# basilevh/tcow

Measured on AMD Instinct MI355X. Metric: train clips/sec (T=30, 240x320), higher is better.
Workload: dtype bf16; 1 GPU; TCOW Seeker train step: T=30 240x320 patch16, 12-layer divided space-time ViT (D=768), num_queries=3, causal_attention=1, 1 clip/GPU; clips_per_gpu=1, num_queries=3, parallelism=dp1, optimizer=AdamW lr 1e-4, clip 0.3

## Files before the change

### include/tcow_hip.h

```cpp
#ifndef TCOW_HIP_H
#define TCOW_HIP_H

#ifdef __cplusplus
extern "C" {
#endif

#define TCOW_OK 0
#define TCOW_ERR_INVALID_ARG (-1)
#define TCOW_ERR_LAUNCH (-2)
#define TCOW_ERR_UNSUPPORTED (-3)

#define TCOW_F32 0
#define TCOW_BF16 1
#define TCOW_F32X3 2

#define TCOW_ACT_NONE 0
#define TCOW_ACT_GELU 1
#define TCOW_ACT_DGELU 2
#define TCOW_ACT_GELU_DSAVE 3
#define TCOW_ACT_MUL_AUX 4

#define TCOW_ABI_VERSION 14
int tcow_version(void);
const char* tcow_last_error(void);
// ... 166 lines not shown
int tcow_droppath_rows(void* stream, int depth, int B, int T, int S, const float* u, const float* keep_p, const float* mask0, float* out);
int tcow_cast_transpose(void* stream, int dtype, int N, int K, const float* W, void* Wc, void* Wt);
long tcow_cast_desc_bytes(void);
int tcow_cast_transpose_batched(void* stream, int dtype, const void* table, int n, int total_tiles);

long tcow_adamw_chunk_bytes(void);
int tcow_adamw_clip_step(void* stream, const void* chunks, int n_chunks, float lr, float beta1, float beta2, float eps,
                         float weight_decay, int step, float max_norm, float* scratch);
int tcow_adamw_clip_step_scaled(void* stream, const void* chunks, int n_chunks, float lr, float beta1, float beta2, float eps,
                                float weight_decay, int step, float max_norm, float* scratch, const float* grad_inv_scale);
long tcow_adamw_tile_bytes(void);
int tcow_adamw_clip_step_cast(void* stream, const void* chunks, int n_chunks, const void* flat_chunks, int n_flat, const void* tiles, int n_tiles, float lr, float beta1,
                              float beta2, float eps, float weight_decay, int step, float max_norm, float* scratch, const float* grad_inv_scale);

typedef struct {
    long n_frames, frame_len, frames_per_seq;
    const float* logits;  long logits_seq_stride;
    const float* target;  long target_seq_stride;
    const float* pixel_w;
    const float* frame_w;
    int weighted_aot;
    float aot_loss;
    double topk_frac;
    float loss_weight;
    float* loss;
    float* total;
    float* dlogits;  long dlogits_seq_stride;
    void* ws;  size_t ws_bytes;
    int focal;
} tcow_mask_loss_args;
size_t tcow_mask_loss_workspace_bytes(long n_frames, long frame_len);
size_t tcow_mask_loss_workspace_bytes_for(long n_frames, long frame_len, double topk_frac, float aot_loss);
int tcow_mask_loss(void* stream, const tcow_mask_loss_args* args);
int tcow_mask_loss_batch(void* stream, const tcow_mask_loss_args* args, int n);

int tcow_iou_counts(void* stream, const float* logits, const float* target, long n_frames, long frame_len, int* counts);

int tcow_build_masks(void* stream, int B, int Q, int M, int T, long HW, int query_time, const unsigned char* segm,
                     const unsigned char* div_segm, const int* query_idx, const int* front_idx, const int* cont_idx,
                     float* query_mask, float* target_mask, unsigned char* snitch_occl_by_ptr, int* counts);

int tcow_build_query_masks(void* stream, int B, int Q, int K, int M, int T, long HW, int query_time, const unsigned char* segm,
                           const unsigned char* div_segm, const float* occl_fracs, const float* dag, const long long* sel, float front_thres,
                           float front_half_thres, float outer_thres, float occluded_weight, float zero_weight, float has_weight, int* idx_ws,
                           unsigned char* ids, float* flags, float* sel_occl_fracs, float* frame_w, float* query_mask, float* target_mask,
                           unsigned char* snitch_occl_by_ptr, int* counts);

int tcow_iou_means(void* stream, const int* counts, int n_seq, int C, int T, float* mean, int* count);

size_t tcow_snitch_weights_workspace_bytes(long n_frames, int H, int W);
int tcow_snitch_weights(void* stream, long n_seq, int T, int H, int W, const float* target_ch0, long target_seq_stride,
                        const unsigned char* snitch_occl_by_ptr, const float* frame_w, const int* pos_count, int class_balancing,
                        float hard_negative_factor, float* weights, void* ws, size_t ws_bytes);

#ifdef __cplusplus
}
#endif
#endif
```

### tcow_amd/_lib.py

```python
import ctypes
import os

_HERE = os.path.dirname(os.path.abspath(__file__))
LIB_PATH = os.environ.get('TCOW_LIB') or os.path.join(_HERE, 'libtcow_hip.so')
LIB_PATH_FP16 = os.path.join(_HERE, 'libtcow_hip_fp16.so')

TCOW_F32, TCOW_BF16, TCOW_F32X3 = 0, 1, 2
TCOW_FP8E4M3 = 3
ACT_NONE, ACT_GELU, ACT_DGELU, ACT_GELU_DSAVE, ACT_MUL_AUX = 0, 1, 2, 3, 4


class TcowError(RuntimeError):
    """Raised when a libtcow_hip entry point returns a non-zero status (message from tcow_last_error)."""


class AttnShape(ctypes.Structure):
    _fields_ = [('B', ctypes.c_int), ('T', ctypes.c_int), ('S', ctypes.c_int), ('D', ctypes.c_int),
                ('heads', ctypes.c_int), ('causal', ctypes.c_int), ('dtype', ctypes.c_int)]


class GemmArgs(ctypes.Structure):
    _fields_ = [('M', ctypes.c_int), ('N', ctypes.c_int), ('K', ctypes.c_int), ('dtype', ctypes.c_int),
                ('A', ctypes.c_void_p), ('lda', ctypes.c_long), ('W', ctypes.c_void_p), ('ldw', ctypes.c_long),
                ('C', ctypes.c_void_p), ('ldc', ctypes.c_long), ('out_f32', ctypes.c_int),
# ... 84 lines not shown
    'tcow_im2col': (_i, [_vp, _i, _i, _i, _i, _i, _i, _vp, _vp, _i, _vp]),
    'tcow_gather_frames': (_i, [_vp, _i, _i, _i, _i, _i, _i, _i, _i, _vp, _vp, _vp, _vp, _vp]),
    'tcow_resize_aa': (_i, [_vp, _i, _i, _i, _i, _i, _i, _i, _i, _i, _vp, _vp, _vp, _vp, _vp, _vp, _vp, _i, _vp, _vp, _vp, _i, _vp]),
    'tcow_photometric_workspace_bytes': (_l, [_i]),
    'tcow_photometric': (_i, [_vp, _i, _i, _i, _i, _i, _i, _i, _i, _vp, _vp, _i, ctypes.POINTER(ctypes.c_int), _f, _f, _f, _f, _i, ctypes.POINTER(ctypes.c_float), _i,
                         _vp, _l, _vp]),
    'tcow_im2col_channels': (_i, [_vp, _i, _i, _i, _i, _i, _i, _i, _vp, _i, _vp]),
    'tcow_col2im': (_i, [_vp, _i, _i, _i, _i, _i, _vp, _l, _vp, _vp, _i, _vp]),
    'tcow_col2im_channels': (_i, [_vp, _i, _i, _i, _i, _i, _i, _vp, _l, _i, _vp, _vp]),
    'tcow_embed_fwd': (_i,[_vp, _i, _i, _i, _i, _vp, _vp, _vp, _vp]),
    'tcow_embed_bwd': (_i, [_vp, _i, _i, _i, _i, _vp, _vp, _vp, _i]),
    'tcow_cls_merge': (_i, [_vp, _i, _i, _i, _i, _vp, _i, _i]),
    'tcow_cls_merge_bwd_cast': (_i, [_vp, _i, _i, _i, _i, _i, _vp, _i, _vp, _l, _vp]),
    'tcow_unpatchify_pool_fwd': (_i, [_vp, _i, _i, _i, _i, _i, _i, _i, _vp, _vp]),
    'tcow_unpatchify_pool_bwd': (_i, [_vp, _i, _i, _i, _i, _i, _i, _i, _vp, _vp]),
    'tcow_upsample_fwd': (_i, [_vp, _i, _i, _i, _i, _i, _i, _i, _vp, _vp]),
    'tcow_upsample_bwd': (_i, [_vp, _i, _i, _i, _i, _i, _i, _i, _vp, _vp]),
    'tcow_upsample_bwd_amax': (_i, [_vp, _i, _i, _i, _i, _i, _i, _vp, _vp, _vp, _i]),
    'tcow_flags_fwd': (_i, [_vp, _i, _i, _i, _i, _vp, _vp, _vp, _vp]),
    'tcow_droppath_rows': (_i, [_vp, _i, _i, _i, _i, _vp, _vp, _vp, _vp]),
    'tcow_scale_cast': (_i, [_vp, _i, _l, _i, _vp, _l, _vp, _vp, _l]),
    'tcow_scale_unless_one': (_i, [_vp, _vp, _l, _vp]),
    'tcow_cast_transpose': (_i, [_vp, _i, _i, _i, _vp, _vp, _vp]),
    'tcow_cast_desc_bytes': (_l, []),
    'tcow_cast_transpose_batched': (_i, [_vp, _i, _vp, _i, _i]),
    'tcow_adamw_chunk_bytes': (_l, []),
    'tcow_adamw_clip_step': (_i, [_vp, _vp, _i, _f, _f, _f, _f, _f, _i, _f, _vp]),
    'tcow_adamw_clip_step_scaled': (_i, [_vp, _vp, _i, _f, _f, _f, _f, _f, _i, _f, _vp, _vp]),
    'tcow_adamw_tile_bytes': (_l, []),
    'tcow_adamw_clip_step_cast': (_i, [_vp, _vp, _i, _vp, _i, _vp, _i, _f, _f, _f, _f, _f, _i, _f, _vp, _vp]),
    'tcow_mask_loss_workspace_bytes': (ctypes.c_size_t, [_l, _l]),
    'tcow_mask_loss_workspace_bytes_for': (ctypes.c_size_t, [_l, _l, ctypes.c_double, _f]),
    'tcow_mask_loss': (_i, [_vp, ctypes.POINTER(MaskLossArgs)]),
    'tcow_mask_loss_batch': (_i, [_vp, ctypes.POINTER(MaskLossArgs), _i]),
    'tcow_iou_counts': (_i, [_vp, _vp, _vp, _l, _l, _vp]),
    'tcow_build_masks': (_i, [_vp, _i, _i, _i, _i, _l, _i, _vp, _vp, _vp, _vp, _vp, _vp, _vp, _vp, _vp]),
    'tcow_build_query_masks': (_i, [_vp, _i, _i, _i, _i, _i, _l, _i, _vp, _vp, _vp, _vp, _vp, _f, _f, _f, _f, _f, _f, _vp, _vp, _vp, _vp, _vp, _vp, _vp, _vp, _vp]),
    'tcow_iou_means': (_i, [_vp, _vp, _i, _i, _i, _vp, _vp]),
    'tcow_snitch_weights_workspace_bytes': (ctypes.c_size_t, [_l, _i, _i]),
    'tcow_snitch_weights': (_i, [_vp, _l, _i, _i, _i, _vp, _l, _vp, _vp, _vp, _i, _f, _vp, _vp, ctypes.c_size_t]),
}


ABI_VERSION = 14


def _declare(L, tolerant=False):
    for name, (res, args) in SIGNATURES.items():
        if tolerant and not hasattr(L, name):
            continue
        fn = getattr(L, name)
        fn.restype = res
        fn.argtypes = args



def lib(fmt='bf16'):
    L = _libs.get(fmt)
    if L is None:
        path = LIB_PATH if fmt == 'bf16' else LIB_PATH_FP16
        if not os.path.exists(path):
            raise TcowError(f'{path} not found: build it with `make` (or __graft_entry__.build()); '
                            'the Seeker HIP path has no fallback')
        import torch
        L = ctypes.CDLL(path)
        L.tcow_last_error.restype = ctypes.c_char_p
# ... 12 lines not shown
```

### tcow_amd/csrc/mask_loss.hip

```cpp
#include "common.h"

namespace {

constexpr int kThreads = 256;
constexpr int kVecPerBlock = 1024;
constexpr int kBins12 = 2048, kBins3 = 512;
constexpr int kNPart = 6;

struct MlView {
    const float* x; long xs;
    const float* t; long ts;
    const float* pw;
    const float* fw;
    float* dx; long dxs;
    int T; int L4; int n_frames; int weighted;
    int focal;
};

struct MlCtl {
    long n_sel, n_all, k, above, cnt_eq, r;
    int valid, mode_all, jac_valid, pad;
    unsigned b1, b2, tau, pad2;
    double S[kNPart];
    double topk_sum;
};

struct MlWs {
    int* fsel; double* fwsum; double* part; unsigned* hist; MlCtl* ctl; int nblk;
    unsigned* vb;
};

constexpr int kMaxJobs = 4;
struct MlJob { MlView v; MlWs ws; float aot, lw; double topk_frac; float* loss; int radix; };
struct MlBatch { int n; float* total; MlJob j[kMaxJobs]; };

__device__ __forceinline__ void bce_sig(float x, float t, float& bce, float& p) {
    const float e = expf(-fabsf(x));
    const float inv = 1.0f / (1.0f + e);
    p = x >= 0.0f ? inv : e * inv;
    bce = fmaxf(x, 0.0f) - x * t + log1pf(e);
}

__device__ __forceinline__ void pix_loss(float x, float t, int focal, float& val, float& dval, float& p) {
    float bce; bce_sig(x, t, bce, p);
    if (!focal) { val = bce; dval = p - t; return; }
    const float pt = p * t + (1.0f - p) * (1.0f - t), at = 0.25f * t + 0.75f * (1.0f - t), q = 1.0f - pt;
    val = at * bce * (q * q);
    dval = at * q * (q * (p - t) - 2.0f * p * (1.0f - p) * (2.0f * t - 1.0f) * bce);
}

__device__ __forceinline__ double block_sum(double v, double* red) {
    for (int o = 32; o > 0; o >>= 1) v += __shfl_xor(v, o, 64);
    const int w = threadIdx.x >> 6;
    __syncthreads();
    if ((threadIdx.x & 63) == 0) red[w] = v;
    __syncthreads();
    double s = 0.0;
    for (int i = 0; i < kThreads / 64; ++i) s += red[i];
    return s;
}

__device__ __forceinline__ long elem_off(const MlView& v, int f, long stride) {
    const int s = f / v.T;
    return (long)s * stride + (long)(f - s * v.T) * v.L4 * 4;
}

__device__ __forceinline__ void ml_frames_body(const MlView& v, const MlWs& ws) {
    __shared__ double red[kThreads / 64];
    const int f = blockIdx.x;
    const float fwv = v.fw ? v.fw[f] : 1.0f;
    double sum = 0.0; int any = 0;
    if (v.pw) {
        const float4* pw = reinterpret_cast<const float4*>(v.pw + (long)f * v.L4 * 4);
        float s = 0.f;
        for (int i = threadIdx.x; i < v.L4; i += kThreads) {
            float4 w = pw[i];
            w.x *= fwv; w.y *= fwv; w.z *= fwv; w.w *= fwv;
            any |= (w.x != 0.f) | (w.y != 0.f) | (w.z != 0.f) | (w.w != 0.f);
            s += (w.x + w.y) + (w.z + w.w);
        }
        sum = s;
    } else if (threadIdx.x == 0) {
        any = fwv != 0.f; sum = (double)fwv * (v.L4 * 4.0);
    }
    sum = block_sum(sum, red);
    any = __syncthreads_or(any);
    if (threadIdx.x == 0) { ws.fsel[f] = any; ws.fwsum[f] = sum; }
}

__device__ __forceinline__ void ml_ctl_body(const MlView& v, const MlWs& ws, double topk_frac) {
    __shared__ double red[kThreads / 64];
    double nf = 0.0, wsum = 0.0;
    for (int f = threadIdx.x; f < v.n_frames; f += kThreads) { nf += ws.fsel[f] ? 1.0 : 0.0; wsum += ws.fwsum[f]; }
    nf = block_sum(nf, red); wsum = block_sum(wsum, red);
    for (int i = threadIdx.x; i < 2 * kBins12 + kBins3; i += kThreads) ws.hist[i] = 0u;
    if (threadIdx.x == 0) {
        MlCtl c = {};
        c.n_all = (long)v.n_frames * v.L4 * 4;
        c.n_sel = (long)nf * v.L4 * 4;
        const float wmean = (float)(wsum / (double)c.n_all);
        c.valid = c.n_sel > 0 && wmean >= 1e-4f;
        c.k = (long)(topk_frac * (double)c.n_sel);
        c.mode_all = c.k >= c.n_sel;
        *ws.ctl = c;
    }
}

template <typename F> __device__ __forceinline__ void for_each_vec(const MlView& v, int f, F&& fn) {
    const float4* x = reinterpret_cast<const float4*>(v.x + elem_off(v, f, v.xs));
    const float4* t = reinterpret_cast<const float4*>(v.t + elem_off(v, f, v.ts));
    const float4* pw = v.pw ? reinterpret_cast<const float4*>(v.pw + (long)f * v.L4 * 4) : nullptr;
    const float fwv = v.fw ? v.fw[f] : 1.0f;
    const int base = blockIdx.x * kVecPerBlock;
#pragma unroll
    for (int j = 0; j < kVecPerBlock / kThreads; ++j) {
        const int i = base + j * kThreads + threadIdx.x;
        if (i < v.L4) {
            float4 w = pw ? pw[i] : make_float4(1.f, 1.f, 1.f, 1.f);
            w.x *= fwv; w.y *= fwv; w.z *= fwv; w.w *= fwv;
            fn(x[i], t[i], w, i);
        }
    }
}

__device__ __forceinline__ unsigned vbits(float bce, float w, int weighted) {
    const unsigned u = __builtin_bit_cast(unsigned, weighted ? bce * w : bce);
    return (int)u < 0 ? 0u : u;
}

__device__ __forceinline__ void ml_stats_body(const MlView& v, const MlWs& ws, int radix) {
    __shared__ unsigned hist[kBins12];
    __shared__ double red[kThreads / 64];
    const int f = blockIdx.y;
    const MlCtl* c = ws.ctl;
    const bool live = c->valid && ws.fsel[f];
    const bool need_hist = live && !c->mode_all && radix;
    if (need_hist) { for (int i = threadIdx.x; i < kBins12; i += kThreads) hist[i] = 0u; }
    __syncthreads();
    float s[5] = {0.f, 0.f, 0.f, 0.f, 0.f};
    if (live) {
        uint4* vbo = need_hist ? reinterpret_cast<uint4*>(ws.vb + (long)f * v.L4 * 4) : nullptr;
        for_each_vec(v, f, [&](float4 x, float4 t, float4 w, int i) {
            const float xs[4] = {x.x, x.y, x.z, x.w}, ts[4] = {t.x, t.y, t.z, t.w}, wv[4] = {w.x, w.y, w.z, w.w};
            unsigned vbs[4];
#pragma unroll
            for (int e = 0; e < 4; ++e) {
                float bce, dval, p; pix_loss(xs[e], ts[e], v.focal, bce, dval, p);
                const unsigned vb = vbits(bce, wv[e], v.weighted);
                vbs[e] = vb;
                s[0] += bce * wv[e]; s[1] += __builtin_bit_cast(float, vb);
                s[2] += p * ts[e]; s[3] += p; s[4] += ts[e];
                if (need_hist) atomicAdd(&hist[vb >> 20], 1u);
            }
            if (vbo) vbo[i] = make_uint4(vbs[0], vbs[1], vbs[2], vbs[3]);
        });
    }
    const int blk = blockIdx.y * gridDim.x + blockIdx.x;
    for (int q = 0; q < 5; ++q) {
        const double tot = block_sum((double)s[q], red);
        if (threadIdx.x == 0) ws.part[(long)blk * kNPart + q] = tot;
    }
    if (need_hist) {
        __syncthreads();
        for (int i = threadIdx.x; i < kBins12; i += kThreads)
            if (hist[i]) atomicAdd(&ws.hist[i], hist[i]);
    }
}

template <int LEVEL> __device__ __forceinline__ void ml_hist_body(const MlView& v, const MlWs& ws) {
    __shared__ unsigned hist[kBins12];
    const int f = blockIdx.y;
    const MlCtl* c = ws.ctl;
    if (!(c->valid && ws.fsel[f]) || c->mode_all) return;
    constexpr int NB = LEVEL == 2 ? kBins12 : kBins3;
    for (int i = threadIdx.x; i < NB; i += kThreads) hist[i] = 0u;
    __syncthreads();
    const unsigned prefix = LEVEL == 2 ? c->b1 : ((c->b1 << 11) | c->b2);
    const uint4* vbi = reinterpret_cast<const uint4*>(ws.vb + (long)f * v.L4 * 4);
    const int base = blockIdx.x * kVecPerBlock;
#pragma unroll
    for (int j = 0; j < kVecPerBlock / kThreads; ++j) {
        const int i = base + j * kThreads + threadIdx.x;
        if (i >= v.L4) continue;
        const uint4 q = vbi[i];
        const unsigned vbs[4] = {q.x, q.y, q.z, q.w};
#pragma unroll
        for (int e = 0; e < 4; ++e) {
            const unsigned vb = vbs[e];
            if (LEVEL == 2) { if ((vb >> 20) == prefix) atomicAdd(&hist[(vb >> 9) & 2047u], 1u); }
            else            { if ((vb >> 9) == prefix) atomicAdd(&hist[vb & 511u], 1u); }
        }
    }
    __syncthreads();
    unsigned* gh = ws.hist + (LEVEL == 2 ? kBins12 : 2 * kBins12);
    for (int i = threadIdx.x; i < NB; i += kThreads)
        if (hist[i]) atomicAdd(&gh[i], hist[i]);
}

template <int LEVEL> __device__ __forceinline__ void ml_scan_body(const MlView& v, const MlWs& ws) {
    __shared__ double red[kThreads / 64];
    MlCtl* c = ws.ctl;
    if (LEVEL == 1) {
        for (int q = 0; q < 5; ++q) {
            double s = 0.0;
            for (int b = threadIdx.x; b < ws.nblk; b += kThreads) s += ws.part[(long)b * kNPart + q];
            s = block_sum(s, red);
            if (threadIdx.x == 0) c->S[q] = s;
        }
        if (threadIdx.x == 0) {
            const float tmean = c->n_sel > 0 ? (float)(c->S[4] / (double)c->n_sel) : 0.f;
            c->jac_valid = !v.weighted && tmean >= 1e-6f;
        }
    }
    if (!c->valid || c->mode_all || threadIdx.x >= 64) return;
    constexpr int NB = LEVEL == 3 ? kBins3 : kBins12;
    constexpr int PER = NB / 64;
    const unsigned* h = ws.hist + (LEVEL == 1 ? 0 : LEVEL == 2 ? kBins12 : 2 * kBins12);
    const long krem = c->k - (LEVEL == 1 ? 0 : c->above);
    const int lane = threadIdx.x;
    long mine = 0;
    for (int i = 0; i < PER; ++i) mine += h[lane * PER + i];
    long incl = mine;
    for (int o = 1; o < 64; o <<= 1) {
        const long up = __shfl_down(incl, o, 64);
        if (lane + o < 64) incl += up;
    }
    const long above_lane = incl - mine;
    if (above_lane < krem && krem <= incl) {
        long acc = above_lane;
        for (int b = lane * PER + PER - 1; b >= lane * PER; --b) {
            const long hb = h[b];
            if (acc + hb >= krem) {
                const long above = (LEVEL == 1 ? 0 : c->above) + acc;
                c->above = above;
                if (LEVEL == 1) c->b1 = (unsigned)b;
                else if (LEVEL == 2) c->b2 = (unsigned)b;
                else { c->tau = (c->b1 << 20) | (c->b2 << 9) | (unsigned)b; c->cnt_eq = hb; c->r = c->k - above; }
                break;
            }
            acc += hb;
        }
    }
}

__device__ __forceinline__ void ml_grad_body(const MlView& v, const MlWs& ws, float aot, float lw) {
    __shared__ double red[kThreads / 64];
    const int f = blockIdx.y;
    const MlCtl* c = ws.ctl;
    const bool live = c->valid && ws.fsel[f];
    float4* dx = v.dx ? reinterpret_cast<float4*>(v.dx + elem_off(v, f, v.dxs)) : nullptr;
    float tk = 0.f;
    if (!live) {
        if (dx) {
            const int base = blockIdx.x * kVecPerBlock;
            for (int j = 0; j < kVecPerBlock / kThreads; ++j) {
                const int i = base + j * kThreads + threadIdx.x;
                if (i < v.L4) dx[i] = make_float4(0.f, 0.f, 0.f, 0.f);
            }
        }
    } else {
        const float sf = lw * sqrtf((float)((double)c->n_sel / (double)c->n_all));
        const float inv_n = (float)(1.0 / (double)c->n_sel);
        const float inv_k = c->k > 0 ? (float)(1.0 / (double)c->k) : 0.f;
        const float c_custom = aot > 0.f ? sf * (1.f - aot) * inv_n : sf * inv_n;
        const float c_boot = aot > 0.f ? sf * aot * (v.weighted ? 1.f : 0.5f) * inv_k : 0.f;
        const float c_jac = (aot > 0.f && c->jac_valid) ? sf * aot * 0.5f : 0.f;
        const float num = (float)c->S[2];
        const float D = (float)(c->S[3] + c->S[4] - c->S[2]) + 0.1f;
// ... 26 lines not shown
__device__ __forceinline__ void ml_final_body(const MlView& v, const MlWs& ws, float aot, float loss_weight, float* loss, float* total) {
    __shared__ double red[kThreads / 64];
    MlCtl* c = ws.ctl;
    double s = 0.0;
    for (int b = threadIdx.x; b < ws.nblk; b += kThreads) s += ws.part[(long)b * kNPart + 5];
    s = block_sum(s, red);
    if (threadIdx.x != 0) return;
    c->topk_sum = s;
    float L = 0.f;
    if (c->valid) {
        const double n = (double)c->n_sel;
        const float custom = (float)(c->S[0] / n);
        if (aot > 0.f) {
            const float boot = c->mode_all ? (float)(c->S[1] / n) : (float)(s / (double)c->k);
            float jac = boot;
            if (!v.weighted) {
                const float num = (float)c->S[2];
                const float den = (float)(c->S[3] + c->S[4] - c->S[2]);
                jac = c->jac_valid ? 1.f - num / (den + 0.1f) : 0.f;
            }
            L = (boot + jac) / 2.f * aot + custom * (1.f - aot);
        } else {
            L = custom;
        }
        L *= sqrtf((float)(n / (double)c->n_all));
    }
    *loss = L;
    if (total) *total += loss_weight * L;
}

__global__ void __launch_bounds__(kThreads) ml_frames_kernel(MlBatch b) { const MlJob& J = b.j[blockIdx.y]; ml_frames_body(J.v, J.ws); }
__global__ void __launch_bounds__(kThreads) ml_ctl_kernel(MlBatch b) { const MlJob& J = b.j[blockIdx.x]; ml_ctl_body(J.v, J.ws, J.topk_frac); }
__global__ void __launch_bounds__(kThreads) ml_stats_kernel(MlBatch b) { const MlJob& J = b.j[blockIdx.z]; ml_stats_body(J.v, J.ws, J.radix); }
template <int LEVEL> __global__ void __launch_bounds__(kThreads) ml_hist_kernel(MlBatch b) { const MlJob& J = b.j[blockIdx.z]; if (J.radix) ml_hist_body<LEVEL>(J.v, J.ws); }
template <int LEVEL> __global__ void __launch_bounds__(kThreads) ml_scan_kernel(MlBatch b) { const MlJob& J = b.j[blockIdx.x]; if (LEVEL == 1 || J.radix) ml_scan_body<LEVEL>(J.v, J.ws); }
__global__ void __launch_bounds__(kThreads) ml_grad_kernel(MlBatch b) { const MlJob& J = b.j[blockIdx.z]; ml_grad_body(J.v, J.ws, J.aot, J.lw); }
__global__ void __launch_bounds__(kThreads) ml_final_kernel(MlBatch b) {
    for (int i = 0; i < b.n; ++i) { const MlJob& J = b.j[i]; ml_final_body(J.v, J.ws, J.aot, J.lw, J.loss, b.total); __syncthreads(); }
}

static int ml_nblk(long n_frames, long frame_len) { return (int)(n_frames * ((frame_len / 4 + kVecPerBlock - 1) / kVecPerBlock)); }

struct MlLayout { size_t fsel, fwsum, part, hist, ctl, vb, total; };
static MlLayout ml_layout(long n_frames, long frame_len, bool radix) {
    const auto pad = [](size_t bytes) { return (bytes + 255) & ~(size_t)255; };
    MlLayout o = {};
    o.fwsum = o.fsel + pad((size_t)n_frames * sizeof(int));
    o.part = o.fwsum + pad((size_t)n_frames * sizeof(double));
    o.hist = o.part + pad((size_t)ml_nblk(n_frames, frame_len) * kNPart * sizeof(double));
    o.ctl = o.hist + (2 * kBins12 + kBins3) * sizeof(unsigned);
    static_assert(sizeof(MlCtl) <= 512, "control block");
    o.vb = o.ctl + 512;
    o.total = o.vb + (radix ? (size_t)n_frames * (size_t)frame_len * sizeof(unsigned) : 0);
    return o;
}
static size_t ml_ws_bytes(long n_frames, long frame_len, bool radix) { return n_frames <= 0 || frame_len <= 0 ? 0 : ml_layout(n_frames, frame_len, radix).total; }

}

extern "C" {

size_t tcow_mask_loss_workspace_bytes(long n_frames, long frame_len) { return ml_ws_bytes(n_frames, frame_len, true); }
size_t tcow_mask_loss_workspace_bytes_for(long n_frames, long frame_len, double topk_frac, float aot_loss) { return ml_ws_bytes(n_frames, frame_len, topk_frac < 1.0 && aot_loss > 0.f); }

static int ml_make_job(const tcow_mask_loss_args* a, MlJob& J) {
    TCOW_CHECK_ARG(a && a->logits && a->target && a->loss && a->ws, "tcow_mask_loss: null argument");
    TCOW_CHECK_ARG(a->n_frames > 0 && a->frame_len > 0 && a->frames_per_seq > 0 && a->n_frames % a->frames_per_seq == 0,
                   "tcow_mask_loss: bad frame counts");
    TCOW_CHECK_ARG(a->frame_len % 4 == 0, "tcow_mask_loss: frame_len %ld must be a multiple of 4", a->frame_len);
    TCOW_CHECK_ARG(a->logits_seq_stride % 4 == 0 && a->target_seq_stride % 4 == 0 && a->dlogits_seq_stride % 4 == 0,
                   "tcow_mask_loss: sequence strides must be multiples of 4 elements");
    TCOW_CHECK_ARG(a->n_frames * (a->frame_len / 4) < (1L << 31) && a->n_frames < 65536, "tcow_mask_loss: too many pixels for one call");
    TCOW_CHECK_ARG(a->topk_frac > 0.0 && a->topk_frac <= 1.0, "tcow_mask_loss: topk_frac %g outside (0, 1]", a->topk_frac);
    TCOW_CHECK_ARG(a->ws_bytes >= tcow_mask_loss_workspace_bytes_for(a->n_frames, a->frame_len, a->topk_frac, a->aot_loss), "tcow_mask_loss: workspace too small");
    MlView& v = J.v;
    v.x = a->logits; v.xs = a->logits_seq_stride; v.t = a->target; v.ts = a->target_seq_stride;
    v.pw = a->pixel_w; v.fw = a->frame_w; v.dx = a->dlogits; v.dxs = a->dlogits_seq_stride;
    v.T = (int)a->frames_per_seq; v.L4 = (int)(a->frame_len / 4); v.n_frames = (int)a->n_frames; v.weighted = a->weighted_aot ? 1 : 0; v.focal = a->focal ? 1 : 0;
    J.aot = a->aot_loss; J.lw = a->loss_weight; J.topk_frac = a->topk_frac; J.loss = a->loss;
    J.radix = (a->topk_frac < 1.0 && a->aot_loss > 0.f) ? 1 : 0;
    const MlLayout o = ml_layout(a->n_frames, a->frame_len, J.radix);
    MlWs& ws = J.ws; char* p = (char*)a->ws;
    ws.fsel = (int*)(p + o.fsel); ws.fwsum = (double*)(p + o.fwsum); ws.part = (double*)(p + o.part); ws.hist = (unsigned*)(p + o.hist);
    ws.ctl = (MlCtl*)(p + o.ctl); ws.vb = (unsigned*)(p + o.vb); ws.nblk = ml_nblk(a->n_frames, a->frame_len);
    return TCOW_OK;
}

int tcow_mask_loss_batch(void* stream, const tcow_mask_loss_args* a, int n) {
    TCOW_CHECK_ARG(a && n >= 1 && n <= kMaxJobs, "tcow_mask_loss_batch: 1 .. %d jobs (got %d)", kMaxJobs, n);
    MlBatch b; b.n = n; b.total = a[0].total;
    int any_radix = 0;
    for (int i = 0; i < n; ++i) {
        const int rc = ml_make_job(a + i, b.j[i]);
        if (rc != TCOW_OK) return rc;
        TCOW_CHECK_ARG(a[i].n_frames == a[0].n_frames && a[i].frame_len == a[0].frame_len && a[i].total == a[0].total,
                       "tcow_mask_loss_batch: the jobs of a batch share n_frames, frame_len and total");
        for (int k = 0; k < i; ++k) TCOW_CHECK_ARG(a[k].ws != a[i].ws, "tcow_mask_loss_batch: every job needs its own workspace");
        any_radix |= b.j[i].radix;
    }
    for (int i = n; i < kMaxJobs; ++i) b.j[i] = b.j[0];
    hipStream_t st = (hipStream_t)stream;
    const MlView& v = b.j[0].v;
    const dim3 grid((v.L4 + kVecPerBlock - 1) / kVecPerBlock, v.n_frames, n);
    ml_frames_kernel<<<dim3(v.n_frames, n), kThreads, 0, st>>>(b);
    ml_ctl_kernel<<<n, kThreads, 0, st>>>(b);
    ml_stats_kernel<<<grid, kThreads, 0, st>>>(b);
    ml_scan_kernel<1><<<n, kThreads, 0, st>>>(b);
    if (any_radix) {
        ml_hist_kernel<2><<<grid, kThreads, 0, st>>>(b);
        ml_scan_kernel<2><<<n, kThreads, 0, st>>>(b);
        ml_hist_kernel<3><<<grid, kThreads, 0, st>>>(b);
        ml_scan_kernel<3><<<n, kThreads, 0, st>>>(b);
    }
    ml_grad_kernel<<<grid, kThreads, 0, st>>>(b);
    ml_final_kernel<<<1, kThreads, 0, st>>>(b);
    TCOW_CHECK_LAUNCH();
    return TCOW_OK;
}

int tcow_mask_loss(void* stream, const tcow_mask_loss_args* a) { return tcow_mask_loss_batch(stream, a, 1); }

}
```

### tcow_amd/ops.py

```python
import ctypes
import threading

import numpy as np
import torch

from . import _lib as L

F32, BF16 = L.TCOW_F32, L.TCOW_BF16
F32X3 = L.TCOW_F32X3
ACT_NONE, ACT_GELU, ACT_DGELU, ACT_GELU_DSAVE, ACT_MUL_AUX = L.ACT_NONE, L.ACT_GELU, L.ACT_DGELU, L.ACT_GELU_DSAVE, L.ACT_MUL_AUX


FP16 = 16


def tdtype(mode):
    return torch.bfloat16 if mode == BF16 else torch.float16 if mode == FP16 else torch.float32


def is16(mode):
    return mode in (BF16, FP16)


def _sel(mode):
# ... 526 lines not shown

def droppath_rows(u, keep_p, mask0, B, T, S):
    _need_cuda(u, keep_p, mask0)
    depth = u.shape[0]
    if u.shape[1] != B * (S - 1) + B * T + B or u.dtype != torch.float32 or not u.is_contiguous() or mask0.numel() != B * T * S:
        raise L.TcowError('droppath_rows: u must be contiguous f32 (depth, B*(S-1) + B*T + B), mask0 [B*T*S]')
    out = torch.empty(4, depth, B * T * S, dtype=torch.float32, device=u.device)
    L.check(L.lib().tcow_droppath_rows(_stream(), depth, B, T, S, u.data_ptr(), keep_p.data_ptr(), mask0.data_ptr(), out.data_ptr()), 'tcow_droppath_rows')
    return out


def cast_transpose(mode, W, Wc=None, Wt=None):
    N, K = W.shape
    lib, dm = _sel(mode)
    L.check(lib.tcow_cast_transpose(_stream(), dm, N, K, W.data_ptr(), _p(Wc), _p(Wt)), 'tcow_cast_transpose', lib)


def cast_transpose_batched(mode, table, n, total_tiles):
    lib, dm = _sel(mode)
    L.check(lib.tcow_cast_transpose_batched(_stream(), dm, table.data_ptr(), int(n), int(total_tiles)), 'tcow_cast_transpose_batched', lib)


def _mask_loss_args(lib, ws_tag, logits, target, channel, pixel_w, frame_w, weighted_aot, aot_loss, topk_frac, loss_weight, loss_out, total, dlogits, focal):
    _need_cuda(logits, target, pixel_w, frame_w, loss_out, total, dlogits)
    BQ, C, T, H, W = logits.shape
    for t in (logits, target, dlogits):
        if t is not None and (t.dtype != torch.float32 or not t.is_contiguous() or t.shape != logits.shape):
            raise L.TcowError('mask_loss: logits / target / dlogits must be contiguous f32 tensors of one shape')
    n_frames, frame_len = BQ * T, H * W
    if pixel_w is not None and (pixel_w.dtype != torch.float32 or not pixel_w.is_contiguous() or pixel_w.numel() != n_frames * frame_len):
        raise L.TcowError('mask_loss: pixel_w must be a contiguous f32 tensor with one weight per pixel')
    if frame_w is not None and (frame_w.dtype != torch.float32 or not frame_w.is_contiguous() or frame_w.numel() != n_frames):
        raise L.TcowError('mask_loss: frame_w must be a contiguous f32 tensor with one weight per frame')
    ws = workspace(lib.tcow_mask_loss_workspace_bytes_for(n_frames, frame_len, float(topk_frac), float(aot_loss)), logits.device, ws_tag)
    off = channel * T * frame_len * 4
    return L.MaskLossArgs(n_frames, frame_len, T, logits.data_ptr() + off, C * T * frame_len, target.data_ptr() + off, C * T * frame_len,
                          _p(pixel_w), _p(frame_w), 1 if weighted_aot else 0, float(aot_loss), float(topk_frac), float(loss_weight),
                          loss_out.data_ptr(), _p(total), (dlogits.data_ptr() + off) if dlogits is not None else None,
                          C * T * frame_len, ws.data_ptr(), ws.numel(), 1 if focal else 0)


def mask_loss(logits, target, channel, pixel_w=None, frame_w=None, weighted_aot=False, aot_loss=0.8, topk_frac=1.0,
              loss_weight=1.0, loss_out=None, total=None, dlogits=None, focal=False):
    lib = L.lib()
    a = _mask_loss_args(lib, 'mask_loss', logits, target, channel, pixel_w, frame_w, weighted_aot, aot_loss, topk_frac, loss_weight, loss_out, total, dlogits, focal)
    L.check(lib.tcow_mask_loss(_stream(), ctypes.byref(a)), 'tcow_mask_loss')
    return loss_out


def mask_loss_channels(logits, target, jobs, aot_loss=0.8, topk_frac=1.0, total=None, dlogits=None, focal=False):
    lib = L.lib()
    arr = (L.MaskLossArgs * len(jobs))()
    for i, (channel, pixel_w, frame_w, weighted_aot, loss_weight, loss_out) in enumerate(jobs):
        arr[i] = _mask_loss_args(lib, 'mask_loss%d' % i, logits, target, channel, pixel_w, frame_w, weighted_aot, aot_loss, topk_frac, loss_weight, loss_out, total,
                                 dlogits, focal)
    L.check(lib.tcow_mask_loss_batch(_stream(), arr, len(jobs)), 'tcow_mask_loss_batch')


def iou_counts(logits, target):
    _need_cuda(logits, target)
    if logits.shape != target.shape or logits.dtype != torch.float32 or target.dtype != torch.float32:
        raise L.TcowError('iou_counts: logits and target must be f32 tensors of one shape')
    lo = logits.contiguous(); tg = target.contiguous()
    frame_len = lo.shape[-1] * lo.shape[-2]
    out = torch.empty(lo.shape[:-2] + (3,), dtype=torch.int32, device=lo.device)
    L.check(L.lib().tcow_iou_counts(_stream(), lo.data_ptr(), tg.data_ptr(), lo.numel() // frame_len, frame_len, out.data_ptr()), 'tcow_iou_counts')
    return out


def _mask_outputs(B, Q, T, H, W, dev):
    return (torch.empty(B, Q, 1, T, H, W, dtype=torch.float32, device=dev), torch.empty(B, Q, 3, T, H, W, dtype=torch.float32, device=dev),
            torch.empty(B, Q, 1, T, H, W, dtype=torch.uint8, device=dev), torch.empty(1 + 2 * Q, dtype=torch.int32, device=dev))


def build_masks(segm, div_segm, query_idx, front_idx, cont_idx, query_time):
    _need_cuda(segm, div_segm, query_idx, front_idx, cont_idx)
    B, _, T, H, W = segm.shape
    M = div_segm.shape[1]; Q = query_idx.shape[1]
    if segm.dtype != torch.uint8 or div_segm.dtype != torch.uint8 or not segm.is_contiguous() or not div_segm.is_contiguous():
        raise L.TcowError('build_masks: segmentation maps must be contiguous uint8 tensors')
# ... 59 lines not shown
```

Baseline: 37.77 clips/s.

## Compact radix top-k candidates into list and use persistent hist grid

During the level-2 radix histogram pass, elements that match the first-level prefix are appended through a shared-memory stage into a global candidate list. The level-3 pass then scans only that list instead of re-reading every value. The hist kernels now run on a persistent grid sized from occupancy, prefetching the next chunk, and the stats reduction and frame-weight sum are batched and unrolled. This adds workspace, atomics and syncs in the level-2 pass. The mask loss is a small part of the ViT training step.

```diff
diff --git a/include/tcow_hip.h b/include/tcow_hip.h
--- a/include/tcow_hip.h
+++ b/include/tcow_hip.h
@@ -222,6 +222,8 @@
 size_t tcow_mask_loss_workspace_bytes(long n_frames, long frame_len);
 size_t tcow_mask_loss_workspace_bytes_for(long n_frames, long frame_len, double topk_frac, float aot_loss);
 int tcow_mask_loss(void* stream, const tcow_mask_loss_args* args);
+size_t tcow_mask_loss_workspace_bytes_with_list(long n_frames, long frame_len, double topk_frac, float aot_loss);
+int tcow_mask_loss_select_info(void* stream, const tcow_mask_loss_args* args, long* info);
 int tcow_mask_loss_batch(void* stream, const tcow_mask_loss_args* args, int n);
 
 int tcow_iou_counts(void* stream, const float* logits, const float* target, long n_frames, long frame_len, int* counts);
diff --git a/tcow_amd/_lib.py b/tcow_amd/_lib.py
--- a/tcow_amd/_lib.py
+++ b/tcow_amd/_lib.py
@@ -140,6 +140,8 @@
     'tcow_mask_loss_workspace_bytes': (ctypes.c_size_t, [_l, _l]),
     'tcow_mask_loss_workspace_bytes_for': (ctypes.c_size_t, [_l, _l, ctypes.c_double, _f]),
     'tcow_mask_loss': (_i, [_vp, ctypes.POINTER(MaskLossArgs)]),
+    'tcow_mask_loss_workspace_bytes_with_list': (ctypes.c_size_t, [_l, _l, ctypes.c_double, _f]),
+    'tcow_mask_loss_select_info': (_i, [_vp, ctypes.POINTER(MaskLossArgs), ctypes.POINTER(ctypes.c_long)]),
     'tcow_mask_loss_batch': (_i, [_vp, ctypes.POINTER(MaskLossArgs), _i]),
     'tcow_iou_counts': (_i, [_vp, _vp, _vp, _l, _l, _vp]),
     'tcow_build_masks': (_i, [_vp, _i, _i, _i, _i, _l, _i, _vp, _vp, _vp, _vp, _vp, _vp, _vp, _vp, _vp]),
diff --git a/tcow_amd/csrc/mask_loss.hip b/tcow_amd/csrc/mask_loss.hip
--- a/tcow_amd/csrc/mask_loss.hip
+++ b/tcow_amd/csrc/mask_loss.hip
@@ -1,3 +1,5 @@
+#include <algorithm>
+
 #include "common.h"
 
 namespace {
@@ -6,6 +8,10 @@
 constexpr int kVecPerBlock = 1024;
 constexpr int kBins12 = 2048, kBins3 = 512;
 constexpr int kNPart = 6;
+constexpr int kVecPerThread = kVecPerBlock / kThreads;
+constexpr unsigned kStage = 6144, kChunkElems = kVecPerBlock * 4;
+constexpr unsigned kStageFlush = kStage - kChunkElems;
+static_assert(kStage > kChunkElems, "stage smaller than a chunk");
 
 struct MlView {
     const float* x; long xs;
@@ -23,11 +29,15 @@
     unsigned b1, b2, tau, pad2;
     double S[kNPart];
     double topk_sum;
+    long n_b1;
+    unsigned cand; int use_list;
 };
 
 struct MlWs {
     int* fsel; double* fwsum; double* part; unsigned* hist; MlCtl* ctl; int nblk;
     unsigned* vb;
+    unsigned* list; unsigned cap;
+    int cpf;
 };
 
 constexpr int kMaxJobs = 4;
@@ -73,12 +83,21 @@
     if (v.pw) {
         const float4* pw = reinterpret_cast<const float4*>(v.pw + (long)f * v.L4 * 4);
         float s = 0.f;
-        for (int i = threadIdx.x; i < v.L4; i += kThreads) {
-            float4 w = pw[i];
+        const auto add = [&](float4 w) {
             w.x *= fwv; w.y *= fwv; w.z *= fwv; w.w *= fwv;
             any |= (w.x != 0.f) | (w.y != 0.f) | (w.z != 0.f) | (w.w != 0.f);
             s += (w.x + w.y) + (w.z + w.w);
-        }
+        };
+        constexpr int U = 8;
+        int i = threadIdx.x;
+        for (; i + (U - 1) * kThreads < v.L4; i += U * kThreads) {
+            float4 w[U];
+#pragma unroll
+            for (int u = 0; u < U; ++u) w[u] = pw[i + u * kThreads];
+#pragma unroll
+            for (int u = 0; u < U; ++u) add(w[u]);
+        }
+        for (; i < v.L4; i += kThreads) add(pw[i]);
         sum = s;
     } else if (threadIdx.x == 0) {
         any = fwv != 0.f; sum = (double)fwv * (v.L4 * 4.0);
@@ -128,9 +147,14 @@
     return (int)u < 0 ? 0u : u;
 }
 
+__device__ __forceinline__ void hist_flush(const unsigned* hist, unsigned* gh, int nb) {
+    for (int i = threadIdx.x; i < nb; i += kThreads)
+        if (hist[i]) atomicAdd(&gh[i], hist[i]);
+}
+
 __device__ __forceinline__ void ml_stats_body(const MlView& v, const MlWs& ws, int radix) {
     __shared__ unsigned hist[kBins12];
-    __shared__ double red[kThreads / 64];
+    __shared__ double red[5][kThreads / 64];
     const int f = blockIdx.y;
     const MlCtl* c = ws.ctl;
     const bool live = c->valid && ws.fsel[f];
@@ -156,55 +180,128 @@
         });
     }
     const int blk = blockIdx.y * gridDim.x + blockIdx.x;
+    double d[5];
+#pragma unroll
     for (int q = 0; q < 5; ++q) {
-        const double tot = block_sum((double)s[q], red);
-        if (threadIdx.x == 0) ws.part[(long)blk * kNPart + q] = tot;
-    }
-    if (need_hist) {
+        d[q] = (double)s[q];
+        for (int o = 32; o > 0; o >>= 1) d[q] += __shfl_xor(d[q], o, 64);
+    }
+    if ((threadIdx.x & 63) == 0) { for (int q = 0; q < 5; ++q) red[q][threadIdx.x >> 6] = d[q]; }
+    __syncthreads();
+    if (threadIdx.x < 5) {
+        double tot = 0.0;
+        for (int i = 0; i < kThreads / 64; ++i) tot += red[threadIdx.x][i];
+        ws.part[(long)blk * kNPart + threadIdx.x] = tot;
+    }
+    if (need_hist) hist_flush(hist, ws.hist, kBins12);
+}
+
+template <int LEVEL> __device__ __forceinline__ void ml_hist_body(const MlView& v, const MlWs& ws) {
+    constexpr int NB = LEVEL == 2 ? kBins12 : kBins3;
+    __shared__ unsigned hist[NB];
+    __shared__ unsigned stage[LEVEL == 2 ? kStage : 1];
+    __shared__ unsigned stage_n, stage_base;
+    MlCtl* c = ws.ctl;
+    if (!c->valid || c->mode_all) return;
+    const bool list = c->use_list != 0;
+    const unsigned prefix = LEVEL == 2 ? c->b1 : ((c->b1 << 11) | c->b2);
+    unsigned* gh = ws.hist + (LEVEL == 2 ? kBins12 : 2 * kBins12);
+    if (LEVEL == 3 && list) {
+        const unsigned cnt = min(c->cand, ws.cap), groups = cnt >> 2;
+        if (blockIdx.x != 0 && blockIdx.x * (unsigned)kThreads >= groups) return;
+        for (int i = threadIdx.x; i < NB; i += kThreads) hist[i] = 0u;
         __syncthreads();
-        for (int i = threadIdx.x; i < kBins12; i += kThreads)
-            if (hist[i]) atomicAdd(&ws.hist[i], hist[i]);
-    }
-}
-
-template <int LEVEL> __device__ __forceinline__ void ml_hist_body(const MlView& v, const MlWs& ws) {
-    __shared__ unsigned hist[kBins12];
-    const int f = blockIdx.y;
-    const MlCtl* c = ws.ctl;
-    if (!(c->valid && ws.fsel[f]) || c->mode_all) return;
-    constexpr int NB = LEVEL == 2 ? kBins12 : kBins3;
+        const uint4* l4 = reinterpret_cast<const uint4*>(ws.list);
+        for (unsigned g = blockIdx.x * kThreads + threadIdx.x; g < groups; g += gridDim.x * kThreads) {
+            const uint4 q = l4[g];
+            const unsigned vbs[4] = {q.x, q.y, q.z, q.w};
+#pragma unroll
+            for (int e = 0; e < 4; ++e)
+                if ((vbs[e] >> 9) == prefix) atomicAdd(&hist[vbs[e] & 511u], 1u);
+        }
+        if (blockIdx.x == 0 && threadIdx.x < (cnt & 3u)) {
+            const unsigned vb = ws.list[groups * 4 + threadIdx.x];
+            if ((vb >> 9) == prefix) atomicAdd(&hist[vb & 511u], 1u);
+        }
+        __syncthreads();
+        hist_flush(hist, gh, NB);
+        return;
+    }
+    const bool append = LEVEL == 2 && list;
     for (int i = threadIdx.x; i < NB; i += kThreads) hist[i] = 0u;
+    if (threadIdx.x == 0) stage_n = 0u;
     __syncthreads();
-    const unsigned prefix = LEVEL == 2 ? c->b1 : ((c->b1 << 11) | c->b2);
-    const uint4* vbi = reinterpret_cast<const uint4*>(ws.vb + (long)f * v.L4 * 4);
-    const int base = blockIdx.x * kVecPerBlock;
-#pragma unroll
-    for (int j = 0; j < kVecPerBlock / kThreads; ++j) {
-        const int i = base + j * kThreads + threadIdx.x;
-        if (i >= v.L4) continue;
-        const uint4 q = vbi[i];
-        const unsigned vbs[4] = {q.x, q.y, q.z, q.w};
-#pragma unroll
-        for (int e = 0; e < 4; ++e) {
-            const unsigned vb = vbs[e];
-            if (LEVEL == 2) { if ((vb >> 20) == prefix) atomicAdd(&hist[(vb >> 9) & 2047u], 1u); }
-            else            { if ((vb >> 9) == prefix) atomicAdd(&hist[vb & 511u], 1u); }
-        }
+    const auto flush_stage = [&](unsigned n) {
+        if (threadIdx.x == 0) stage_base = atomicAdd(&c->cand, n);
+        __syncthreads();
+        const unsigned b = stage_base;
+        for (unsigned i = threadIdx.x; i < n; i += kThreads)
+            if (b + i < ws.cap) ws.list[b + i] = stage[i];
+        if (threadIdx.x == 0) stage_n = 0u;
+        __syncthreads();
+    };
+    const auto fetch = [&](int q, uint4 (&in)[kVecPerThread]) {
+        const int f = q / ws.cpf, base = (q - f * ws.cpf) * kVecPerBlock;
+        const uint4* vbi = reinterpret_cast<const uint4*>(ws.vb + (long)f * v.L4 * 4);
+        const bool live = ws.fsel[f] != 0;
+#pragma unroll
+        for (int j = 0; j < kVecPerThread; ++j) {
+            const int i = base + j * kThreads + threadIdx.x;
+            in[j] = make_uint4(~0u, ~0u, ~0u, ~0u);
+            if (live && i < v.L4) in[j] = vbi[i];
+        }
+    };
+    uint4 in[kVecPerThread], ahead[kVecPerThread];
+    if ((int)blockIdx.x < ws.nblk) fetch(blockIdx.x, in);
+    for (int q = blockIdx.x; q < ws.nblk; q += gridDim.x) {
+        if (q + (int)gridDim.x < ws.nblk) fetch(q + gridDim.x, ahead);
+#pragma unroll
+        for (int j = 0; j < kVecPerThread; ++j) {
+            const unsigned vbs[4] = {in[j].x, in[j].y, in[j].z, in[j].w};
+#pragma unroll
+            for (int e = 0; e < 4; ++e) {
+                const unsigned vb = vbs[e];
+                if (LEVEL == 2) {
+                    const bool m = (vb >> 20) == prefix;
+                    if (m) atomicAdd(&hist[(vb >> 9) & 2047u], 1u);
+                    if (append) {
+                        const unsigned long long bal = __ballot(m);
+                        if (bal) {
+                            const int lane = threadIdx.x & 63, lead = __ffsll((long long)bal) - 1;
+                            unsigned at = 0u;
+                            if (lane == lead) at = atomicAdd(&stage_n, (unsigned)__popcll(bal));
+                            at = __shfl(at, lead, 64);
+                            if (m) stage[at + __popcll(bal & ((1ull << lane) - 1ull))] = vb;
+                        }
+                    }
+                } else if ((vb >> 9) == prefix) atomicAdd(&hist[vb & 511u], 1u);
+            }
+        }
+        if (append) {
+            __syncthreads();
+            const unsigned n = stage_n;
+            if (n > kStageFlush) flush_stage(n); else __syncthreads();
+        }
+#pragma unroll
+        for (int j = 0; j < kVecPerThread; ++j) in[j] = ahead[j];
     }
     __syncthreads();
-    unsigned* gh = ws.hist + (LEVEL == 2 ? kBins12 : 2 * kBins12);
-    for (int i = threadIdx.x; i < NB; i += kThreads)
-        if (hist[i]) atomicAdd(&gh[i], hist[i]);
+    if (append && stage_n > 0u) { const unsigned n = stage_n; __syncthreads(); flush_stage(n); }
+    hist_flush(hist, gh, NB);
 }
 
 template <int LEVEL> __device__ __forceinline__ void ml_scan_body(const MlView& v, const MlWs& ws) {
     __shared__ double red[kThreads / 64];
     MlCtl* c = ws.ctl;
     if (LEVEL == 1) {
+        double s5[5] = {0.0, 0.0, 0.0, 0.0, 0.0};
+        for (int b = threadIdx.x; b < ws.nblk; b += kThreads) {
+#pragma unroll
+            for (int q = 0; q < 5; ++q) s5[q] += ws.part[(long)b * kNPart + q];
+        }
+#pragma unroll
         for (int q = 0; q < 5; ++q) {
-            double s = 0.0;
-            for (int b = threadIdx.x; b < ws.nblk; b += kThreads) s += ws.part[(long)b * kNPart + q];
-            s = block_sum(s, red);
+            const double s = block_sum(s5[q], red);
             if (threadIdx.x == 0) c->S[q] = s;
         }
         if (threadIdx.x == 0) {
@@ -233,7 +330,7 @@
             if (acc + hb >= krem) {
                 const long above = (LEVEL == 1 ? 0 : c->above) + acc;
                 c->above = above;
-                if (LEVEL == 1) c->b1 = (unsigned)b;
+                if (LEVEL == 1) { c->b1 = (unsigned)b; c->n_b1 = hb; c->use_list = hb <= (long)ws.cap; }
                 else if (LEVEL == 2) c->b2 = (unsigned)b;
                 else { c->tau = (c->b1 << 20) | (c->b2 << 9) | (unsigned)b; c->cnt_eq = hb; c->r = c->k - above; }
                 break;
@@ -326,7 +423,7 @@
 __global__ void __launch_bounds__(kThreads) ml_frames_kernel(MlBatch b) { const MlJob& J = b.j[blockIdx.y]; ml_frames_body(J.v, J.ws); }
 __global__ void __launch_bounds__(kThreads) ml_ctl_kernel(MlBatch b) { const MlJob& J = b.j[blockIdx.x]; ml_ctl_body(J.v, J.ws, J.topk_frac); }
 __global__ void __launch_bounds__(kThreads) ml_stats_kernel(MlBatch b) { const MlJob& J = b.j[blockIdx.z]; ml_stats_body(J.v, J.ws, J.radix); }
-template <int LEVEL> __global__ void __launch_bounds__(kThreads) ml_hist_kernel(MlBatch b) { const MlJob& J = b.j[blockIdx.z]; if (J.radix) ml_hist_body<LEVEL>(J.v, J.ws); }
+template <int LEVEL> __global__ void __launch_bounds__(kThreads) ml_hist_kernel(MlBatch b) { const MlJob& J = b.j[blockIdx.y]; if (J.radix) ml_hist_body<LEVEL>(J.v, J.ws); }
 template <int LEVEL> __global__ void __launch_bounds__(kThreads) ml_scan_kernel(MlBatch b) { const MlJob& J = b.j[blockIdx.x]; if (LEVEL == 1 || J.radix) ml_scan_body<LEVEL>(J.v, J.ws); }
 __global__ void __launch_bounds__(kThreads) ml_grad_kernel(MlBatch b) { const MlJob& J = b.j[blockIdx.z]; ml_grad_body(J.v, J.ws, J.aot, J.lw); }
 __global__ void __launch_bounds__(kThreads) ml_final_kernel(MlBatch b) {
@@ -335,7 +432,17 @@
 
 static int ml_nblk(long n_frames, long frame_len) { return (int)(n_frames * ((frame_len / 4 + kVecPerBlock - 1) / kVecPerBlock)); }
 
-struct MlLayout { size_t fsel, fwsum, part, hist, ctl, vb, total; };
+template <typename K> static int ml_resident(K kernel) {
+    int dev = 0, cus = 0, per = 0;
+    if (hipGetDevice(&dev) != hipSuccess || hipDeviceGetAttribute(&cus, hipDeviceAttributeMultiprocessorCount, dev) != hipSuccess ||
+        hipOccupancyMaxActiveBlocksPerMultiprocessor(&per, kernel, kThreads, 0) != hipSuccess || cus <= 0 || per <= 0) { (void)hipGetLastError(); return 2048; }
+    return cus * per;
+}
+static dim3 ml_grid(int nblk, int n_jobs, int resident) {
+    return dim3((unsigned)std::min(nblk, std::max(1, resident / n_jobs)), n_jobs);
+}
+
+struct MlLayout { size_t fsel, fwsum, part, hist, ctl, vb, total, list; };
 static MlLayout ml_layout(long n_frames, long frame_len, bool radix) {
     const auto pad = [](size_t bytes) { return (bytes + 255) & ~(size_t)255; };
     MlLayout o = {};
@@ -346,8 +453,10 @@
     static_assert(sizeof(MlCtl) <= 512, "control block");
     o.vb = o.ctl + 512;
     o.total = o.vb + (radix ? (size_t)n_frames * (size_t)frame_len * sizeof(unsigned) : 0);
+    o.list = (o.total + 15) & ~(size_t)15;
     return o;
 }
+static size_t ml_list_entries(long n_frames, long frame_len) { return (size_t)n_frames * (size_t)frame_len / 4; }
 static size_t ml_ws_bytes(long n_frames, long frame_len, bool radix) { return n_frames <= 0 || frame_len <= 0 ? 0 : ml_layout(n_frames, frame_len, radix).total; }
 
 }
@@ -356,6 +465,11 @@
 
 size_t tcow_mask_loss_workspace_bytes(long n_frames, long frame_len) { return ml_ws_bytes(n_frames, frame_len, true); }
 size_t tcow_mask_loss_workspace_bytes_for(long n_frames, long frame_len, double topk_frac, float aot_loss) { return ml_ws_bytes(n_frames, frame_len, topk_frac < 1.0 && aot_loss > 0.f); }
+size_t tcow_mask_loss_workspace_bytes_with_list(long n_frames, long frame_len, double topk_frac, float aot_loss) {
+    const bool radix = topk_frac < 1.0 && aot_loss > 0.f;
+    if (n_frames <= 0 || frame_len <= 0 || !radix) return ml_ws_bytes(n_frames, frame_len, radix);
+    return ml_layout(n_frames, frame_len, true).list + ml_list_entries(n_frames, frame_len) * sizeof(unsigned);
+}
 
 static int ml_make_job(const tcow_mask_loss_args* a, MlJob& J) {
     TCOW_CHECK_ARG(a && a->logits && a->target && a->loss && a->ws, "tcow_mask_loss: null argument");
@@ -377,6 +491,9 @@
     MlWs& ws = J.ws; char* p = (char*)a->ws;
     ws.fsel = (int*)(p + o.fsel); ws.fwsum = (double*)(p + o.fwsum); ws.part = (double*)(p + o.part); ws.hist = (unsigned*)(p + o.hist);
     ws.ctl = (MlCtl*)(p + o.ctl); ws.vb = (unsigned*)(p + o.vb); ws.nblk = ml_nblk(a->n_frames, a->frame_len);
+    ws.cpf = ws.nblk / v.n_frames;
+    const size_t spare = J.radix && a->ws_bytes > o.list ? (a->ws_bytes - o.list) / sizeof(unsigned) : 0;
+    ws.list = (unsigned*)(p + o.list); ws.cap = (unsigned)std::min(std::min(spare, (size_t)a->n_frames * (size_t)a->frame_len), (size_t)0xFFFFFFFFu);
     return TCOW_OK;
 }
 
@@ -395,15 +512,18 @@
     for (int i = n; i < kMaxJobs; ++i) b.j[i] = b.j[0];
     hipStream_t st = (hipStream_t)stream;
     const MlView& v = b.j[0].v;
+    static const int res_hist = ml_resident(ml_hist_kernel<2>);
+    const int nblk = b.j[0].ws.nblk;
     const dim3 grid((v.L4 + kVecPerBlock - 1) / kVecPerBlock, v.n_frames, n);
+    const dim3 grid_hist = ml_grid(nblk, n, res_hist);
     ml_frames_kernel<<<dim3(v.n_frames, n), kThreads, 0, st>>>(b);
     ml_ctl_kernel<<<n, kThreads, 0, st>>>(b);
     ml_stats_kernel<<<grid, kThreads, 0, st>>>(b);
     ml_scan_kernel<1><<<n, kThreads, 0, st>>>(b);
     if (any_radix) {
-        ml_hist_kernel<2><<<grid, kThreads, 0, st>>>(b);
+        ml_hist_kernel<2><<<grid_hist, kThreads, 0, st>>>(b);
         ml_scan_kernel<2><<<n, kThreads, 0, st>>>(b);
-        ml_hist_kernel<3><<<grid, kThreads, 0, st>>>(b);
+        ml_hist_kernel<3><<<grid_hist, kThreads, 0, st>>>(b);
         ml_scan_kernel<3><<<n, kThreads, 0, st>>>(b);
     }
     ml_grad_kernel<<<grid, kThreads, 0, st>>>(b);
@@ -414,4 +534,18 @@
 
 int tcow_mask_loss(void* stream, const tcow_mask_loss_args* a) { return tcow_mask_loss_batch(stream, a, 1); }
 
-}
+int tcow_mask_loss_select_info(void* stream, const tcow_mask_loss_args* a, long* info) {
+    TCOW_CHECK_ARG(info, "tcow_mask_loss_select_info: null argument");
+    MlJob J;
+    const int rc = ml_make_job(a, J);
+    if (rc != TCOW_OK) return rc;
+    MlCtl c;
+    hipError_t e = hipMemcpyAsync(&c, J.ws.ctl, sizeof(c), hipMemcpyDeviceToHost, (hipStream_t)stream);
+    if (e == hipSuccess) e = hipStreamSynchronize((hipStream_t)stream);
+    if (e != hipSuccess) { tcow_set_error("tcow_mask_loss_select_info: %s", hipGetErrorString(e)); return TCOW_ERR_LAUNCH; }
+    const bool ran = J.radix && c.valid && !c.mode_all;
+    info[0] = ran ? c.use_list : 0; info[1] = ran ? c.n_b1 : 0; info[2] = ran ? (long)c.cand : 0; info[3] = (long)J.ws.cap;
+    return TCOW_OK;
+}
+
+}
diff --git a/tcow_amd/ops.py b/tcow_amd/ops.py
--- a/tcow_amd/ops.py
+++ b/tcow_amd/ops.py
@@ -582,7 +582,10 @@
         raise L.TcowError('mask_loss: pixel_w must be a contiguous f32 tensor with one weight per pixel')
     if frame_w is not None and (frame_w.dtype != torch.float32 or not frame_w.is_contiguous() or frame_w.numel() != n_frames):
         raise L.TcowError('mask_loss: frame_w must be a contiguous f32 tensor with one weight per frame')
-    ws = workspace(lib.tcow_mask_loss_workspace_bytes_for(n_frames, frame_len, float(topk_frac), float(aot_loss)), logits.device, ws_tag)
+    need = lib.tcow_mask_loss_workspace_bytes_for(n_frames, frame_len, float(topk_frac), float(aot_loss))
+    pin = _scratch.pinned.get(ws_tag)
+    ws = pin if pin is not None and pin.numel() >= need else \
+        workspace(lib.tcow_mask_loss_workspace_bytes_with_list(n_frames, frame_len, float(topk_frac), float(aot_loss)), logits.device, ws_tag)
     off = channel * T * frame_len * 4
     return L.MaskLossArgs(n_frames, frame_len, T, logits.data_ptr() + off, C * T * frame_len, target.data_ptr() + off, C * T * frame_len,
                           _p(pixel_w), _p(frame_w), 1 if weighted_aot else 0, float(aot_loss), float(topk_frac), float(loss_weight),
@@ -596,6 +599,15 @@
     a = _mask_loss_args(lib, 'mask_loss', logits, target, channel, pixel_w, frame_w, weighted_aot, aot_loss, topk_frac, loss_weight, loss_out, total, dlogits, focal)
     L.check(lib.tcow_mask_loss(_stream(), ctypes.byref(a)), 'tcow_mask_loss')
     return loss_out
+
+
+def mask_loss_select_info(logits, target, channel, aot_loss=0.8, topk_frac=1.0, ws_tag='mask_loss'):
+    lib = L.lib()
+    dummy = torch.zeros(1, dtype=torch.float32, device=logits.device)
+    a = _mask_loss_args(lib, ws_tag, logits, target, channel, None, None, False, aot_loss, topk_frac, 1.0, dummy, None, None, False)
+    info = (ctypes.c_long * 4)()
+    L.check(lib.tcow_mask_loss_select_info(_stream(), ctypes.byref(a), info), 'tcow_mask_loss_select_info')
+    return dict(list_used=bool(info[0]), prefix_count=int(info[1]), appended=int(info[2]), capacity=int(info[3]))
 
 
 def mask_loss_channels(logits, target, jobs, aot_loss=0.8, topk_frac=1.0, total=None, dlogits=None, focal=False):
```

Result: no change. 37.68 clips/s (-0.2%).
